# caltech-netlab/adacharge

Hardware: AMD Instinct MI355X
Metric: MPC QP solves/sec whole-node, 54 EVSE x horizon 12; max rate residual vs cvxpy (higher is better)
Workload: dtype f64; 1 GPU; caltech54 (Caltech-shaped, 54 EVSE) x horizon 12, quick_charge + equal_share*1e-12, SOC constraints, batches of 256 independent MPC snapshots (BASELINE.json configs[1]); one step = one acnqp_solve_batches call over 64 such batches per GPU (16384 problems), pinned host buffers in, host buffers out: H2D + kernels + D2H inside the timed region; batch=256, n_evse=54, horizon=12, constraint_type=SOC, parallelism=dp1 (own snapshots per GPU)

## Files before the change

adacharge_amd/backend.py:

```python
from __future__ import annotations

import ctypes as C
import dataclasses
import os
from dataclasses import dataclass
from typing import Optional

import numpy as np

from .builder import CONE_SOC, ProblemBatch, SiteData

_LIB_NAME = "libacn_qp_hip.so"
_LIB_DIR = os.path.join(os.path.dirname(os.path.abspath(__file__)), "lib")

STATUS_UNSET = 0
STATUS_SOLVED = 1
STATUS_MAX_ITER = 2
STATUS_PRIMAL_INFEASIBLE = 3
STATUS_EMPTY_SET = 4
STATUS_SOLVED_INACCURATE = 5
ACCEPTED_STATUSES = (STATUS_SOLVED, STATUS_SOLVED_INACCURATE)
STATUS_NAMES = {
    STATUS_UNSET: "unset",
    STATUS_SOLVED: "optimal",
# ... 122 lines not shown
        ("acnqp_ordered_launch_count", i64, [h]),
        ("acnqp_polish_stats", rc, [h, P(i64), i32]),
        ("acnqp_accel_columns", i32, [h, i32, i32, i32, i32]),
        ("acnqp_route", i32, [h, i32, i32, i32, P(i32)]),
    ]
    for stem, args in (
        ("acnqp_duals", [h, P(_Problems), P(Options), ptr, ptr, ptr, P(_Duals)]),
        ("acnqp_pilots", [h, P(_PilotPlan), ptr, P(_Pilots)]),
        ("acnqp_advance", advance + [P(_Next), ptr]),
        ("acnqp_advance_priced", advance + [P(ClockCost), P(_Next), ptr]),
        ("acnqp_prepare", [h, P(_Problems), P(_PreparePlan), ptr, ptr, P(_PrepareView), ptr]),
    ):
        rows += [(stem + "_host", rc, args), (stem + "_device", rc, args + [stream])]
    introspection = [
        ("acnqp_debug_polish_alongside", i64, [h]),
        ("acnqp_debug_wave_rank", rc, [h, P(i32)]),
        ("acnqp_debug_wave_evse_extent", rc, [h, P(i32)]),
        ("acnqp_debug_order_keys", rc, [h, P(_Problems), P(i32)]),
        ("acnqp_debug_copy_workspace", i64, [h, ptr, i64]),
    ]
    return tuple(r + (True,) for r in rows) + tuple(r + (False,) for r in introspection)


_ABI = _abi()
EXPORTED_SYMBOLS = tuple(name for name, _, _, declared in _ABI if declared)

_lib = None


def library_path() -> str:
# ... 380 lines not shown
        want_y = [False] * n if want_y is None else list(want_y)
        warm = [None] * n if warm is None else list(warm)
        if len(want_y) != n or len(warm) != n:
            raise ValueError("want_y and warm need one entry per batch")
        P, R = (_Problems * n)(), (_Results * n)()
        results, keep = [], []
        for g, batch in enumerate(batches):
            self._check_site(batch)
            P[g], R[g], res, k = self._marshal(batch, pinned_results, warm=warm[g], want_y=bool(want_y[g]))
            results.append(res)
            keep.append(k)
        _check(self._lib.acnqp_solve_batches(self._h, n, P, C.byref(o), R), "acnqp_solve_batches")
        del keep
        return [self._finish(b, r) for b, r in zip(batches, results)]

    def prepare_many(self, batches, pinned_results: bool = True, x_dev_ptrs=None):
        n = len(batches)
        P, R = (_Problems * n)(), (_Results * n)()
        results, keep = [], []
        for g, batch in enumerate(batches):
            self._check_site(batch)
            P[g], R[g], res, k = self._marshal(batch, pinned_results, None if x_dev_ptrs is None else x_dev_ptrs[g])
            results.append(res)
            keep.append(k)

        def run(options: Options):
            _check(self._lib.acnqp_solve_batches(self._h, n, P, C.byref(options), R), "acnqp_solve_batches")
            return results

        run.keep = keep
        return run, results

    def solve_device(self, dev: "DeviceBatch", options: Optional[Options] = None, stream: int = 0, warm_x=None, warm_y=None) -> None:
        o = options if options is not None else default_options()
        if (warm_x is None) != (warm_y is None):
            raise ValueError("warm_x and warm_y go together (both or neither)")
        _want(warm_x, "warm_x", _F8, (dev.B, dev.N, dev.Tm))
# ... 198 lines not shown
        return dict(rank=int(buf[0]), eig_ksteps=int(buf[1]), extent=int(buf[2]))

    def wave_evse_extent(self) -> dict:
        buf = (C.c_int32 * 3)()
        if self._lib.acnqp_debug_wave_evse_extent(self._h, buf) != 0:
            raise RuntimeError("acnqp_debug_wave_evse_extent failed")
        return dict(n_evse=int(buf[0]), evse_ksteps=int(buf[1]), extent=int(buf[2]))

    def order_keys(self, dev: "DeviceBatch") -> np.ndarray:
        keys = np.empty(dev.B, np.int32)
        p = _device_problems(dev)
        if self._lib.acnqp_debug_order_keys(self._h, C.byref(p), keys.ctypes.data_as(C.POINTER(C.c_int32))) != 0:
            raise RuntimeError("acnqp_debug_order_keys failed")
        return keys

    def ordered_launches(self) -> int:
        return int(self._lib.acnqp_ordered_launch_count(self._h))

    def last_kernel_ms(self) -> float:
        return float(self._lib.acnqp_last_kernel_ms(self._h))

    def kernel_times(self, capacity: int = 64):
        buf = (C.c_float * int(capacity))()
        n = int(self._lib.acnqp_kernel_times(self._h, buf, int(capacity)))
        return [float(buf[k]) for k in range(n)]

    def route(self, t_max: int, k_sessions: int, batch: int = 1):
        pol = C.c_int32(0)
        fam = int(self._lib.acnqp_route(self._h, int(t_max), int(k_sessions), int(batch), C.byref(pol)))
        if fam == 0:
# ... 47 lines not shown
```

adacharge_amd/csrc/acn_qp_api.hip:

```cpp
#include <hip/hip_runtime.h>

#include <algorithm>
#include <chrono>
#include <cmath>
#include <cstdint>
#include <cstdio>
#include <cstdlib>
#include <cstring>
#include <initializer_list>
#include <string>
#include <vector>

#include "acn_qp.h"
#include "acn_qp_launch.hpp"
#include "acn_qp_duals.hpp"
#include "acn_qp_pilots.hpp"
#include "acn_qp_advance.hpp"
#include "acn_qp_prepare.hpp"
#include "acn_qp_site.hpp"

namespace {

thread_local std::string g_last_error;

// ... 46 lines not shown
    cap = 0;
  }
};

}

struct acnqp_handle {
  int device = 0;
  acnqp::SiteShape shape;
  std::vector<double> G, limits;
  acnqp::SiteDev site;
  static constexpr int kEvRing = 64;
  hipEvent_t ev_start[kEvRing] = {}, ev_stop[kEvRing] = {};
  long long launches = 0, reported = 0;
  long long ordered_launches = 0;
  static constexpr int kSlots = 4;
  struct Slot { hipStream_t st = nullptr; DevBuf in, out, tin; } slot[kSlots];
  HostBuf small_in, small_out;
  hipEvent_t h2d_done[kSlots] = {nullptr, nullptr, nullptr, nullptr};
  struct Work {
    hipStream_t st; DevBuf buf; DevBuf ord; DevBuf pol; long long used; hipEvent_t last; DevBuf dua;
    hipEvent_t fork = nullptr, join = nullptr;
    void release_events() {
      if (last) (void)hipEventDestroy(last);
      if (fork) (void)hipEventDestroy(fork);
      if (join) (void)hipEventDestroy(join);
      last = fork = join = nullptr;
    }
  };
  std::vector<Work> work;
// ... 79 lines not shown
  static long long stream_workspace(int NP, int CT, int K, int MT, int accel) { return acnqp::stream_workspace(NP, CT, K, MT, accel); }
  static long long long_workspace(int NP, int t_max, int K, int MT, int accel) { return acnqp::long_workspace(NP, acnqp::long_tiles(t_max), K, MT, accel); }
};

int polish_block_doubles(const acnqp_handle* h, const acnqp::Route& rt) {
  static const bool no_polish = std::getenv("ACNQP_NO_POLISH") != nullptr;
  if (no_polish || !rt.polish_shape) return -1;
  const acnqp::SiteShape& s = h->shape;
  const int nrow_site = s.M + s.has_peak;
  const bool two_per_cu = rt.tiled && rt.t_max <= 16 && s.MR == 16 && rt.k_sessions == 1;
  const int blk = acnqp::polish_blocks_that_fit(s.N, rt.t_max, s.Mg, nrow_site, acnqp::polish_max_sess(s.N, rt.k_sessions),
                                                two_per_cu ? 76 * 1024 : 160 * 1024);
  return blk < 2 * nrow_site * (2 * nrow_site + 1) / 2 ? -1 : blk;
}

int solve_batch_device(acnqp_handle* h, const acnqp_problems* p, const acnqp_options* o, acnqp_results* r, hipStream_t st, bool nothing_follows);

}

#include "acn_qp_pipeline.hpp"
#include "acn_qp_post.hpp"
extern "C" {

int32_t acnqp_abi_version(void) { return ACNQP_ABI_VERSION; }

int32_t acnqp_route(acnqp_handle* h, int32_t t_max, int32_t k_sessions, int32_t batch, int32_t* polish) {
  if (polish) *polish = 0;
  if (!h || t_max < 1 || t_max > 4096 || k_sessions < 1 || k_sessions > 4096 || batch < 1) return 0;
  const acnqp::Route r = route_of(h, t_max, k_sessions, batch);
  acnqp_options o;
  acnqp_default_options(&o);
// ... 166 lines not shown
  a.x = r->x; a.status = r->status; a.iters = r->iters; a.pri = r->pri_res; a.dua = r->dua_res; a.obj = r->obj;
  a.eps_abs = o->eps_abs; a.eps_rel = o->eps_rel; a.rho0 = o->rho; a.sigma = o->sigma; a.alpha = o->alpha;
  a.adapt_tol = o->adapt_tol; a.reg_rel = o->reg_rel;
  a.max_iter = o->max_iter; a.check_every = o->check_every; a.adapt_every = o->adapt_every;
  a.peak_scale = d->peak_scale; a.flat_scale = d->flat_scale; a.max_scale = d->max_scale;
  a.accel_mem = std::max(0, o->accel_mem);
  a.stall_iters = o->stall_iters; a.retry_passes = o->retry_passes; a.retry_max_iter = o->retry_max_iter;
  a.retry_rho = o->retry_rho; a.inacc_floor = o->inaccurate_floor;
  a.pbuf_single = 0;
  a.order = nullptr;
  a.queue = nullptr;
  bool own = false;
  for (auto& sl : h->slot) own = own || sl.st == st;
  a.grid_oversub = own ? 4 : 1;
  a.polish_iters = 0; a.polish_stall = 0; a.resume = 0; a.y_for_polish_only = 0; a.pol_rows = 0; a.pol_list = nullptr; a.pol_count = nullptr; a.pol_retired = nullptr; a.count_dev = nullptr;
  return a;
}

hipError_t launch_order_keys(acnqp_handle* h, const acnqp::Route& rt, const acnqp_problems* p, hipStream_t st, int32_t* keys) {
  static const bool by_sessions = [] { const char* e = std::getenv("ACNQP_ORDER_KEY"); return e && std::strcmp(e, "sessions") == 0; }();
  const acnqp::SiteShape& s = h->shape;
  const int g_rows = s.cone == ACNQP_CONE_SOC ? 2 * s.M : s.M;
  const int waves = by_sessions || rt.family == ACNQP_ROUTE_WAVE4 ? 0 : order_key_waves((size_t)s.N, (size_t)p->t_max, (size_t)g_rows);
  if (waves == 0) {
    hipLaunchKernelGGL(session_keys_kernel, dim3((p->batch + 3) / 4), dim3(256), 0, st, p->s_len, p->k_sessions * s.N, p->batch, keys);
    return hipGetLastError();
  }
  OrderKeyArgs ka;
  ka.B = p->batch; ka.N = s.N; ka.Tm = p->t_max; ka.K = p->k_sessions; ka.M = s.M; ka.soc = s.cone == ACNQP_CONE_SOC; ka.has_peak = s.has_peak;
  ka.lb = p->lb; ka.ub = p->ub; ka.s_cap = p->s_cap; ka.peak = p->peak; ka.G = h->site.Gabi; ka.limits = h->site.limabi;
// ... 62 lines not shown
    w.Ghat = h->site.GhatW; w.lam = h->site.lamW; w.fragQ = h->site.fragQW; w.extent = wave_extent_of(h);
    w.evse_ksteps = wave_evse_extent_of(h);
    return acnqp::launch_wave(aa, w, st);
  }
  if (rt.tiled) return rt.t_max <= 16 ? acnqp::launch_tiled_ct1(aa, st) : acnqp::launch_tiled_ct2(aa, st);
  if (rt.stream || rt.lng) {
    acnqp::StreamArgs sa;
    sa.t = aa; sa.work = static_cast<double*>(ws.p); sa.ws_per_problem = ws.per_problem;
    return rt.stream ? acnqp::launch_stream(sa, st) : acnqp::launch_long(sa, st, rt.lds);
  }
  const long long nvar = (long long)rt.site.N * rt.t_max;
  const int nt = nvar <= 4096 ? 256 : (nvar <= 12288 ? 512 : 1024);
  acnqp::GeneralArgs ga;
  ga.t = aa; ga.work = ws.p; ga.ws_per_problem = ws.per_problem; ga.pair_stride = 4;
  return acnqp::launch_general(ga, nt, st);
}

int launch_with_polish(acnqp_handle* h, acnqp_handle::Work* wk, const acnqp::Route& rt, const acnqp::TiledArgs& a, const Workspace& ws,
                       int pol_blk, const acnqp_problems* p, const acnqp_options* o, const acnqp_results* r, hipStream_t st, bool nothing_follows,
                       hipError_t* e) {
  static const bool no_alongside = std::getenv("ACNQP_NO_POLISH_ALONGSIDE") != nullptr;
  static const long long along_polls = [] {
    const char* v = std::getenv("ACNQP_POLISH_ALONGSIDE_SPINS");
    const long long n = v ? std::atoll(v) : (1ll << 21);
    return n < 0 ? 0ll : n;
  }();
  static const int along_grid = [] {
    const char* v = std::getenv("ACNQP_POLISH_ALONGSIDE_GRID");
    const int n = v ? std::atoi(v) : 0;
    return n > 0 && n <= 256 ? n : 16;
// ... 40 lines not shown
    pa.alongside = 0; pa.expected = p->batch; pa.retired = ctr + 3; pa.max_polls = along_polls; pa.taken = h->pol_stats + 16;
    if (alongside) {
      acnqp::PolishArgs pc = pa;
      pc.alongside = 1;
      HIP_TRY(hipStreamWaitEvent(h->aux, wk->fork, 0));
      *e = acnqp::launch_polish(pc, along_grid, h->aux);
      HIP_TRY(hipEventRecord(wk->join, h->aux));
      HIP_TRY(hipStreamWaitEvent(st, wk->join, 0));
    }
    if (*e == hipSuccess) *e = acnqp::launch_polish(pa, pol_grid, st);
  }
  if (*e == hipSuccess) {
    acnqp::TiledArgs a3 = a;
    a3.resume = 1; a3.order = list; a3.count_dev = ctr + 2; a3.queue = ctr + 1;
    a3.warm_x = r->x; a3.warm_y = ybuf;
    a3.ws_by_slot = 1; a3.grid_cap = std::min(p->batch, a.grid_oversub > 1 ? 64 : 2 * h->cus);
    if (!a.ws_by_slot) a3.grid_cap = std::min(a3.grid_cap, a.grid_cap);
    *e = launch_solver(h, rt, a3, ws, st);
  }
  return ACNQP_OK;
}

int solve_batch_device(acnqp_handle* h, const acnqp_problems* p, const acnqp_options* o, acnqp_results* r, hipStream_t st, bool nothing_follows) {
  int rc = check_problem_shapes(h, p, o, r);
  if (rc != ACNQP_OK) return rc;
  if (p->batch == 0) return ACNQP_OK;
  HIP_TRY(hipSetDevice(h->device));
  acnqp::TiledArgs a = tiled_args(h, p, o, r, st);
  (void)hipGetLastError();
  HIP_TRY(hipMemsetAsync(r->status, 0, (size_t)p->batch * sizeof(int32_t), st));
  const int evk = (int)(h->launches % acnqp_handle::kEvRing);
  HIP_TRY(hipEventRecord(h->ev_start[evk], st));
  const acnqp::Route rt = route_of(h, p->t_max, p->k_sessions, p->batch);
  acnqp_handle::Work* wk = h->work_for(st);
  if ((rc = schedule_launch(h, wk, rt, p, st, &a)) != ACNQP_OK) return rc;
  Workspace ws;
  if ((rc = reserve_workspace(wk, rt, st, &a, &ws)) != ACNQP_OK) return rc;
  const int pol_blk = (o->polish_iters > 0 && o->polish_iters < o->max_iter && !a.warm_x) ? polish_block_doubles(h, rt) : -1;
  hipError_t e = hipSuccess;
  if (pol_blk >= 0) {
    if ((rc = launch_with_polish(h, wk, rt, a, ws, pol_blk, p, o, r, st, nothing_follows, &e)) != ACNQP_OK) return rc;
  } else {
    e = launch_solver(h, rt, a, ws, st);
  }
  if (e != hipSuccess) return fail(ACNQP_ERR_HIP, std::string("kernel launch: ") + hipGetErrorString(e));
  HIP_TRY(hipEventRecord(h->ev_stop[evk], st));
  if (wk->last) HIP_TRY(hipEventRecord(wk->last, st));
  ++h->launches;
// ... 29 lines not shown
  HIP_TRY(hipSetDevice(h->device));
  HIP_TRY(hipDeviceSynchronize());
  int32_t v[16] = {0};
  HIP_TRY(hipMemcpy(v, h->pol_stats, sizeof(v), hipMemcpyDeviceToHost));
  for (int k = 0; k < capacity && k < 16; ++k) out[k] = v[k];
  return ACNQP_OK;
}

extern "C" int64_t acnqp_debug_polish_alongside(acnqp_handle* h) {
  if (!h || hipSetDevice(h->device) != hipSuccess || hipDeviceSynchronize() != hipSuccess) return -1;
  int32_t v = 0;
  if (hipMemcpy(&v, h->pol_stats + 16, sizeof v, hipMemcpyDeviceToHost) != hipSuccess) return -1;
  if (hipMemset(h->pol_stats + 16, 0, sizeof v) != hipSuccess) return -1;
  return v;
}

extern "C" int acnqp_debug_wave_rank(acnqp_handle* h, int32_t* out) {
  if (!h || !out) return -1;
  const int ext = wave_extent_of(h);
  out[0] = h->site.rank; out[1] = h->site.eig_ksteps; out[2] = ext > 0 ? ext : h->shape.MR / 4;
  return 0;
}

extern "C" int acnqp_debug_order_keys(acnqp_handle* h, const acnqp_problems* p, int32_t* keys_out) {
  if (!h || !p || !keys_out || p->batch < 0 || p->t_max < 1 || p->k_sessions < 1) return -1;
  if (p->batch == 0) return 0;
  if (!p->lb || !p->ub || !p->s_off || !p->s_len || !p->s_cap || !p->horizon) return -1;
  if (hipSetDevice(h->device) != hipSuccess) return -1;
  int32_t* keys = nullptr;
  if (hipMalloc((void**)&keys, (size_t)p->batch * sizeof(int32_t)) != hipSuccess) return -1;
// ... 128 lines not shown
```

adacharge_amd/csrc/acn_qp_common.hpp:

```cpp
#pragma once
#include <hip/hip_runtime.h>
#include <stdint.h>

#include "acn_qp_check.hpp"

namespace acnqp {

#ifdef ACNQP_STAMPS
__device__ unsigned long long g_stamps[1024 * 16 * 12];
#define STAMP(slot)                                                                    \
  do {                                                                                 \
    unsigned long long _t;                                                             \
    __builtin_amdgcn_sched_barrier(0);                                                 \
    asm volatile("s_memtime %0\n\ts_waitcnt lgkmcnt(0)" : "=s"(_t)::"memory");         \
    __builtin_amdgcn_sched_barrier(0);                                                 \
    st_acc[slot] += _t - st_prev;                                                      \
    st_prev = _t;                                                                      \
  } while (0)
#else
#define STAMP(slot) do {} while (0)
#endif

#ifndef ACNQP_GUARD_MAX
#define ACNQP_GUARD_MAX 120
// ... 26 lines not shown
  double *pri, *dua, *obj;
  double eps_abs, eps_rel, rho0, sigma, alpha, adapt_tol, reg_rel;
  double peak_scale, flat_scale, max_scale;
  int max_iter, check_every, adapt_every;
  int accel_mem;
  int stall_iters, retry_passes, retry_max_iter;
  double inacc_floor, retry_rho;
  int pbuf_single;
  int polish_iters, resume;
  int polish_stall;
  int y_for_polish_only;
  int pol_rows;
  int32_t *pol_list, *pol_count;
  int32_t* pol_retired;
  const int32_t* count_dev;
  int ws_by_slot;
  int grid_oversub;
  int grid_cap;
};

typedef const __attribute__((address_space(4))) TiledArgs* KernargPtr;

__device__ inline int queue_length(const TiledArgs& a) {
  if (a.count_dev == nullptr) return a.B;
  const int n = *a.count_dev;
  return n < a.B ? n : a.B;
}
__device__ inline int queue_next(int32_t* queue, int B, int round, int* slot_lds) {
  if (queue == nullptr) return round == 0 && (int)blockIdx.x < B ? (int)blockIdx.x : -1;
  if (threadIdx.x == 0) *slot_lds = atomicAdd(queue, 1);
// ... 160 lines not shown
```

adacharge_amd/csrc/acn_qp_pipeline.hpp:

```cpp
#pragma once
#include <algorithm>
#include <cstddef>
#include <cstdlib>
#include <vector>

namespace acnqp {

inline size_t al256(size_t b) { return (b + 255) & ~(size_t)255; }

struct ChunkLayout {
  size_t lb, ub, q, pd, hz, so, sl, sc, eq, pk, lf, dc, df, wx, wy, in_total;
  size_t x, st, it, pr, du, ob, y, out_total;
  ChunkLayout(size_t cn, size_t N, size_t Tm, size_t K, size_t Mg, bool peak, bool flat, bool mx, bool warm, bool want_y) {
    size_t o = 0;
    lb = o; o += al256(cn * N * Tm * 8);
    ub = o; o += al256(cn * N * Tm * 8);
    q = o;  o += al256(cn * N * Tm * 8);
    pd = o; o += al256(cn * 8);
    hz = o; o += al256(cn * 4);
    so = o; o += al256(cn * K * N * 4);
    sl = o; o += al256(cn * K * N * 4);
    sc = o; o += al256(cn * K * N * 8);
    eq = o; o += al256(cn);
    pk = o; o += al256(peak ? cn * Tm * 8 : 0);
    lf = o; o += al256(flat ? cn * 8 : 0);
    dc = o; o += al256(mx ? cn * 8 : 0);
    df = o; o += al256(mx ? cn * 8 : 0);
    wx = o; o += al256(warm ? cn * N * Tm * 8 : 0);
    wy = o; o += al256(warm ? cn * Mg * Tm * 8 : 0);
    in_total = o;
    o = 0;
    x = o;  o += al256(cn * N * Tm * 8);
    st = o; o += al256(cn * 4);
    it = o; o += al256(cn * 4);
    pr = o; o += al256(cn * 8);
    du = o; o += al256(cn * 8);
    ob = o; o += al256(cn * 8);
    y = o;  o += al256(want_y ? cn * Mg * Tm * 8 : 0);
    out_total = o;
  }
};

struct PlanEnv {
  long long chunk = 0;
  const char* plan = nullptr;
  bool ramp = true;
};

inline long long chunk_cap_by_memory(size_t N, size_t Tm, size_t K) {
  const size_t per_problem = 4 * N * Tm * 8 + K * N * 16 + Tm * 8 + 96;
  return (long long)((size_t)1024 * 1024 * 1024 / std::max<size_t>(per_problem, 1));
}

inline std::vector<long long> plan_chunk_caps(long long total, long long want, long long by_mem, bool wave, bool uniform,
                                              const PlanEnv& env) {
  if (env.chunk > 0) want = env.chunk;
  long long cap = std::max<long long>(1, std::min(want, by_mem));
  if (cap >= 512) cap -= cap % 512;
  std::vector<long long> caps;
  if (env.ramp && wave && uniform) {
    if (env.plan) {
      for (const char* q = env.plan; *q;) { caps.push_back(std::max<long long>(1, std::atoll(q))); while (*q && *q != ',') ++q; if (*q == ',') ++q; }
    } else if (total >= 2048 && cap >= 2048) {
      const long long k = (total + cap - 1) / cap - 1;
      long long c = total / (k + 1);
      c = std::max<long long>(2048, std::min(cap, c - c % 512));
      caps.push_back(c / 4);
      caps.push_back(c / 2);
      for (long long i = 0; i < k; ++i) caps.push_back(c);
    }
    caps.push_back(std::max<long long>(1, total));
  } else if (env.ramp && cap >= 1024) {
    caps = {cap / 4, cap / 2, cap};
  } else {
    caps = {cap};
  }
  return caps;
// ... 176 lines not shown
    qt = o; o += al256((size_t)T->n_horizons * nv * 8);
    total = o;
  }
};

struct BatchShape { long long batch; int t_max, k_sessions; bool warm, want_y; };
struct Piece { int g; long long lo, n, pos; };
struct Scatter { int g; size_t lo, n, pos; const char* host; size_t st, it, pr, du, ob; };

struct Call {
  const acnqp_problems* P = nullptr;
  const acnqp_table* T = nullptr;
  acnqp_results* R = nullptr;
  std::vector<BatchShape> bs;
  std::vector<Scatter> scatter;
};

void device_views(const ChunkLayout& L, char* di, char* dq, const acnqp::SiteShape& s, size_t cn, const BatchShape& b,
                  acnqp_problems* dp, acnqp_results* dr) {
  dp->batch = (int32_t)cn; dp->t_max = b.t_max; dp->k_sessions = b.k_sessions;
  dp->lb = reinterpret_cast<const double*>(di + L.lb);
  dp->ub = reinterpret_cast<const double*>(di + L.ub);
  dp->q = reinterpret_cast<const double*>(di + L.q);
  dp->pdiag = reinterpret_cast<const double*>(di + L.pd);
  dp->horizon = reinterpret_cast<const int32_t*>(di + L.hz);
  dp->s_off = reinterpret_cast<const int32_t*>(di + L.so);
  dp->s_len = reinterpret_cast<const int32_t*>(di + L.sl);
  dp->s_cap = reinterpret_cast<const double*>(di + L.sc);
  dp->s_eq = reinterpret_cast<const uint8_t*>(di + L.eq);
  dp->peak = s.has_peak ? reinterpret_cast<const double*>(di + L.pk) : nullptr;
  dp->lf = s.has_flat ? reinterpret_cast<const double*>(di + L.lf) : nullptr;
// ... 18 lines not shown
    total += b.batch;
    uniform = uniform && b.t_max == bs[0].t_max && b.k_sessions == bs[0].k_sessions && b.warm == bs[0].warm && b.want_y == bs[0].want_y;
  }
  std::vector<std::vector<Piece>> chunks;
  std::vector<long long> caps;
  long long fill = 0, cap = 0;
  const BatchShape* cur = nullptr;
  for (int g = 0; g < (int)bs.size(); ++g) {
    const BatchShape& b = bs[g];
    for (long long lo = 0; lo < b.batch;) {
      if (!cur || b.t_max != cur->t_max || b.k_sessions != cur->k_sessions || b.warm != cur->warm || b.want_y != cur->want_y || fill >= cap) {
        chunks.emplace_back();
        cur = &b; fill = 0;
        if (caps.empty() || !uniform) {
          const acnqp::Route rt = acnqp::route_for(h->shape, b.t_max, b.k_sessions, (int)std::min<long long>(total, acnqp::kRouteAnyBatch), route_switches());
          caps = acnqp::plan_chunk_caps(total, rt.chunk_want(), acnqp::chunk_cap_by_memory((size_t)h->shape.N, (size_t)b.t_max, (size_t)b.k_sessions),
                                        rt.wv > 0, uniform, env);
        }
        cap = acnqp::chunk_cap(caps, chunks.size() - 1);
      }
      const long long n = std::min(b.batch - lo, cap - fill);
      chunks.back().push_back({g, lo, n, fill});
      fill += n; lo += n;
    }
  }
  return chunks;
}

int fill_dense(acnqp_handle* h, const Call& call, size_t c, const std::vector<Piece>& pcs, const ChunkLayout& L,
               acnqp_handle::Slot& S, char* hs) {
  const acnqp::SiteShape& s = h->shape;
  const BatchShape& b = call.bs[pcs[0].g];
// ... 13 lines not shown
    else H2D(field, base, elem, per);                                                                           \
  } while (0)
    H2D(lb, L.lb, 8, nv);
    H2D(ub, L.ub, 8, nv);
    H2D(q, L.q, 8, nv);
    H2S(pdiag, L.pd, 8, 1);
    H2S(horizon, L.hz, 4, 1);
    H2S(s_off, L.so, 4, ns);
    H2S(s_len, L.sl, 4, ns);
    H2S(s_cap, L.sc, 8, ns);
    H2S(s_eq, L.eq, 1, 1);
    if (s.has_peak) H2S(peak, L.pk, 8, Tm);
    if (s.has_flat) H2S(lf, L.lf, 8, 1);
    if (s.has_max) { H2S(dc, L.dc, 8, 1); H2S(dfloor, L.df, 8, 1); }
    if (b.warm) { H2D(warm_x, L.wx, 8, nv); H2D(warm_y, L.wy, 8, Mg * Tm); }
#undef H2S
#undef H2D
  }
  if (hs) HIP_TRY(hipMemcpyAsync(di + L.pd, hs + L.pd, L.wx - L.pd, hipMemcpyHostToDevice, S.st));
  if (chain) HIP_TRY(hipEventRecord(h->h2d_done[c % acnqp_handle::kSlots], S.st));
  return ACNQP_OK;
}

int fill_table(acnqp_handle* h, const Call& call, const Piece& pc, const ChunkLayout& L, const TableLayout& TL, acnqp_handle::Slot& S) {
  const acnqp::SiteShape& s = h->shape;
  const acnqp_table* T = call.T;
  const size_t N = s.N, Tm = T->t_max, K = T->k_sessions, nv = N * Tm;
  const long long lo = pc.lo, cn = pc.n, s0 = TL.s0, ns = TL.ns, r0 = TL.r0, nr = TL.nr;
  char* di = static_cast<char*>(S.in.p);
  char* dt = static_cast<char*>(S.tin.p);
// ... 27 lines not shown
  ea.lb = reinterpret_cast<double*>(di + L.lb); ea.ub = reinterpret_cast<double*>(di + L.ub); ea.q = reinterpret_cast<double*>(di + L.q);
  ea.so = reinterpret_cast<int32_t*>(di + L.so); ea.sl = reinterpret_cast<int32_t*>(di + L.sl); ea.sc = reinterpret_cast<double*>(di + L.sc);
  hipLaunchKernelGGL(table_expand_kernel, dim3((unsigned)cn), dim3(256), 0, S.st, ea);
  return ACNQP_OK;
}

int run_call(acnqp_handle* h, Call& call, const acnqp_options* o) {
  const acnqp::SiteShape& s = h->shape;
  const size_t N = s.N, Mg = s.Mg;
  const bool table = call.T != nullptr;
  acnqp::PlanEnv env;
  if (const char* e = std::getenv("ACNQP_CHUNK")) env.chunk = std::atoll(e);
  env.plan = std::getenv("ACNQP_PLAN");
  static const bool ramp = std::getenv("ACNQP_NO_RAMP") == nullptr;
  env.ramp = ramp;
  const std::vector<std::vector<Piece>> chunks = split_call(h, call.bs, env);
  auto layout = [&](const std::vector<Piece>& pcs) {
    const BatchShape& b = call.bs[pcs[0].g];
    return ChunkLayout((size_t)(pcs.back().pos + pcs.back().n), N, b.t_max, b.k_sessions, Mg, s.has_peak, s.has_flat, s.has_max, b.warm, b.want_y);
  };
  constexpr size_t kSmallCap = (size_t)256 << 20;
  std::vector<size_t> in_off(chunks.size()), out_off(chunks.size());
  size_t in_sum = 0, out_sum = 0;
  for (size_t c = 0; c < chunks.size() && !table; ++c) {
    const ChunkLayout L = layout(chunks[c]);
    in_off[c] = in_sum; in_sum += L.wx - L.pd;
    out_off[c] = out_sum; out_sum += L.y - L.st;
  }
  static const bool no_stage = std::getenv("ACNQP_NO_STAGING") != nullptr;
  const bool staged = !table && !no_stage && in_sum + out_sum <= kSmallCap;
  if (staged) {
    HIP_TRY(h->small_in.reserve(in_sum));
    HIP_TRY(h->small_out.reserve(out_sum));
  }
  for (size_t c = 0; c < chunks.size(); ++c) {
    acnqp_handle::Slot& S = h->slot[c % acnqp_handle::kSlots];
    const std::vector<Piece>& pcs = chunks[c];
    const BatchShape& b = call.bs[pcs[0].g];
    const size_t cn = (size_t)(pcs.back().pos + pcs.back().n), Tm = b.t_max;
    const ChunkLayout L = layout(pcs);
    const TableLayout TL = table ? TableLayout(call.T, pcs[0].lo, pcs[0].n, N * Tm) : TableLayout();
    if (L.in_total > S.in.cap || L.out_total > S.out.cap || TL.total > S.tin.cap) HIP_TRY(hipStreamSynchronize(S.st));
    HIP_TRY(S.in.reserve(L.in_total));
    HIP_TRY(S.out.reserve(L.out_total));
    if (table) HIP_TRY(S.tin.reserve(TL.total));
    char* di = static_cast<char*>(S.in.p);
    char* dq = static_cast<char*>(S.out.p);
    char* hs = staged ? static_cast<char*>(h->small_in.p) + in_off[c] - L.pd : nullptr;
    char* ho = staged ? static_cast<char*>(h->small_out.p) + out_off[c] - L.st : nullptr;
    int rc = table ? fill_table(h, call, pcs[0], L, TL, S) : fill_dense(h, call, c, pcs, L, S, hs);
    if (rc != ACNQP_OK) return rc;
    acnqp_problems dp;
    acnqp_results dr;
    device_views(L, di, dq, s, cn, b, &dp, &dr);
    rc = solve_batch_device(h, &dp, o, &dr, S.st, c + 1 == chunks.size());
    if (rc != ACNQP_OK) return rc;
    if (staged) HIP_TRY(hipMemcpyAsync(ho + L.st, dq + L.st, L.y - L.st, hipMemcpyDeviceToHost, S.st));
    for (const Piece& pc : pcs) {
      const acnqp_results& r = call.R[pc.g];
      const size_t lo = (size_t)pc.lo, n = (size_t)pc.n, pos = (size_t)pc.pos;
#define D2H(field, base, elem, per)                                                                          \
  HIP_TRY(hipMemcpyAsync(reinterpret_cast<char*>(r.field) + lo * (per) * (elem), dq + (base) + pos * (per) * (elem), \
                         n * (per) * (elem), hipMemcpyDeviceToHost, S.st))
      D2H(x, L.x, 8, N * Tm);
      if (staged) {
        call.scatter.push_back(Scatter{pc.g, lo, n, pos, ho, L.st, L.it, L.pr, L.du, L.ob});
      } else {
        D2H(status, L.st, 4, 1);
        D2H(iters, L.it, 4, 1);
        D2H(pri_res, L.pr, 8, 1);
        D2H(dua_res, L.du, 8, 1);
        D2H(obj, L.ob, 8, 1);
      }
      if (b.want_y) D2H(y, L.y, 8, Mg * Tm);
#undef D2H
      if (r.x_dev)
        HIP_TRY(hipMemcpyAsync(r.x_dev + lo * N * Tm, dq + L.x + pos * N * Tm * 8, n * N * Tm * 8, hipMemcpyDeviceToDevice, S.st));
    }
  }
// ... 38 lines not shown
```

adacharge_amd/csrc/acn_qp_route.hpp:

```cpp
#pragma once
#include <algorithm>

#include "acn_qp.h"

namespace acnqp {

constexpr int kRouteMaxK = 4;
constexpr int kRouteWaveTS = 12;

inline int padded_rows(int cone, int M, int has_peak, int has_flat, int has_max) {
  return (cone == ACNQP_CONE_SOC ? 8 * ((M + 3) / 4) : M) + (has_peak ? 1 : 0) + (has_flat ? 1 : 0) + (has_max ? 1 : 0);
}

struct SiteShape {
  int N = 0, M = 0, Mg = 0, MR = 0;
  int cone = 0, has_peak = 0, has_flat = 0, has_max = 0;
  int NP() const { return N <= 64 ? 64 : 16 * ((N + 15) / 16); }
};

inline SiteShape site_shape(int N, int M, int cone, int has_peak, int has_flat, int has_max) {
  SiteShape s;
  s.N = N; s.M = M; s.cone = cone;
  s.has_peak = has_peak ? 1 : 0; s.has_flat = has_flat ? 1 : 0; s.has_max = has_max ? 1 : 0;
  s.Mg = (cone == ACNQP_CONE_SOC ? 2 * M : M) + s.has_peak + s.has_flat + s.has_max;
// ... 31 lines not shown
inline bool stream_shape(const SiteShape& s, int t_max) { return s.N > 64 && t_max <= 48; }
inline bool long_shape(const SiteShape& s, int t_max, int k_sessions, const RouteSwitches& sw) {
  return !sw.no_long && !tiled_shape(s, t_max, k_sessions) && !stream_shape(s, t_max) && t_max <= 288 && s.MR <= 32;
}

struct Route {
  int family = 0;
  int wv = 0;
  bool tiled = false, stream = false, lng = false, lds = false, on_chip = false;
  bool polish_shape = false;
  SiteShape site;
  int t_max = 0, k_sessions = 0;

  long long chunk_want() const { return wv > 0 ? 8192 : (tiled ? 1024 : 2048); }

  template <class Kn> int accel_cap() const {
    if (wv > 0) return Kn::wave_accel();
    if (tiled) return Kn::tiled_accel(site.MR / 16, (t_max + 15) / 16, site.NP(), k_sessions);
    if (stream) return Kn::stream_accel();
    if (lng) return Kn::long_accel();
    return Kn::general_accel();
  }

  template <class Kn> long long workspace_doubles(int accel_req) const {
    if (tiled) return 0;
    const int accel = std::min(std::max(0, accel_req), accel_cap<Kn>());
    if (stream) return Kn::stream_workspace(site.NP(), (t_max + 15) / 16, k_sessions, site.MR / 16, accel);
    if (lng) return Kn::long_workspace(site.NP(), t_max, k_sessions, site.MR / 16, accel);
    const long long n = (long long)site.N * t_max, mt = (long long)site.MR * t_max, Dn = n + mt;
    return 7 * n + 8 * mt + 3LL * k_sessions * site.N + 8 + 2 * Dn + ((1 + 2LL * accel) * Dn * 4 + 7) / 8 + 2;
// ... 26 lines not shown
```

adacharge_amd/csrc/acn_qp_wave.hpp:

```cpp
#pragma once
#include <type_traits>

#include "acn_qp_common.hpp"

namespace acnqp {

constexpr int kWaveTS = 12;
constexpr int kWaveXS = 17;
constexpr int kWaveNW = 4;
constexpr int kWaveAM = 5;

struct WaveLds {
  int fragp, fragx, fragq, rowc, wave0, wstride;
  int xt, rowd, aah, snap, hist, total;
  int xch;
  int xs;
  __host__ __device__ WaveLds(int accel_mem, int npw = 1, int mt = 1, int tsv = kWaveTS) {
    int o = 0;
    fragp = o; o += mt * 16 * 64;
    fragx = o; o += 4 * 4 * mt * 64;
    fragq = o; o += mt * mt * 2 * 4 * 64;
    rowc = o;  o += mt * (16 + 16 + 8);
    wave0 = o;
    int w = 0;
// ... 16 lines not shown
    const int pos = (int)blockIdx.x * kWaveNW + wave;
    return round == 0 && pos < B ? pos : -1;
  }
  int v = 0;
  if (lane == 0) v = atomicAdd(queue, 1);
  const int pos = __builtin_amdgcn_readfirstlane(v);
  return pos < B ? pos : -1;
}

__device__ inline void wave_lds_sync() {
  __builtin_amdgcn_fence(__ATOMIC_RELEASE, "wavefront");
  __builtin_amdgcn_wave_barrier();
  __builtin_amdgcn_fence(__ATOMIC_ACQUIRE, "wavefront");
}

template <int AM, int NPW, int TSV, int MT, bool PROX, int EK = 0, int NE = 0>
__global__ __launch_bounds__(kWaveNW * 64, 1) void admm_wave_kernel(const TiledArgs A_kernarg) {
  static_assert(NPW == 1 || NPW == 2 || NPW == 4, "one, two or four waves per problem");
  static_assert((TSV == 12 && MT == 1) || (TSV == 6 && MT == 2 && NPW >= 2), "instantiated: 12 periods x one row tile, 6 periods x two row tiles");
  using M = Mfma<double>;
  using vec4 = typename M::vec4;
  typedef double real;
  constexpr int TS = TSV, XS = TSV > 8 ? kWaveXS : 9, XC = TSV > 8 ? 16 : 8;
  constexpr int SR = 4 * MT, KS = 4 * MT;
  constexpr int EKS = EK > 0 ? EK : KS, ET = (EKS + 3) / 4;
  static_assert(EKS <= KS, "eigen extent");
  constexpr int NKS = NE > 0 ? NE : 16;
  static_assert(NKS <= 16, "EVSE extent");
#define EKOF(m) (EKS - 4 * (m) < 4 ? EKS - 4 * (m) : 4)
#define BIGC (scalar_const(1e300))
// ... 291 lines not shown
#pragma unroll
    for (int t = 0; t < TS; ++t) {
      f1 = fmax(f1, fabs(qv[t]));
      f2 = fmax(f2, ubv[t]);
      if (!((swm >> t) & 1u)) f3 = fmax(f3, fmax(fabs(lbv[t]), fabs(ubv[t])));
    }
    f1 = wave_max<real>(f1); f2 = wave_max<real>(f2); f3 = wave_max<real>(f3);
    { real f[3] = {f1, f2, f3}; pu_max(f, 3); f1 = f[0]; f2 = f[1]; f3 = f[2]; }
    plain_windows = uniform_scalar(f3) == 0.0;
    qnorm = uniform_scalar(f1);
    pd = uniform_scalar(effective_pdiag<real>(pd_user, A.reg_rel, qnorm, uniform_scalar(f2), A.horizon[b], PROX && ((lfb > 0.0) | (dcb > 0.0))));
    if (__any(empty_set)) {
#pragma unroll
      for (int t = 0; t < TS; ++t)
        if (act && tb + t < Tm) A.x[((size_t)b * N + lane) * Tm + tb + t] = 0;
      if (A.y_out && !A.y_for_polish_only && half == 0)
        for (int k = lane; k < A.Mg * Tm; k += 64) A.y_out[(size_t)b * A.Mg * Tm + k] = 0;
      if (lane == 0 && half == 0) {
        A.status[b] = 4; A.iters[b] = 0;
        A.pri[b] = 1e300; A.dua[b] = 1e300; A.obj[b] = 0;
      }
      break;
    }
  }

  real z2[SR], y2[SR], gx[SR];
#pragma unroll
  for (int r = 0; r < SR; ++r) { z2[r] = 0; y2[r] = 0; gx[r] = 0; }

  rho = uniform_scalar(rho);
// ... 655 lines not shown
    STAMP(7);
  }
  it_total += it;
  if (lane == 0 && half == 0) A.iters[b] = it_total;
  if (pass == 0 || status_rank(status) > status_rank(best_status)) {
    best_status = status;
    real ol = 0;
    int lane_o = lane;
    asm volatile("" : "+v"(lane_o));
#pragma unroll
    for (int t = 0; t < TS; ++t)
      if (lane_o < N && tb + t < Tm) {
        A.x[((size_t)b * N + lane_o) * Tm + tb + t] = z1[t];
        ol += (0.5 * pd_user * z1[t] + qv[t]) * z1[t];
      }
    if (A.y_out && (!A.y_for_polish_only || status == kStatusPolish)) {
      const real* RS = static_cast<const real*>(A.rowscale);
      const int g_o = lane_o >> 4, t_o = lane_o & 15;
#pragma unroll
      for (int r = 0; r < SR; ++r) {
        const int j = 16 * (r >> 2) + M::rowof(g_o, r & 3);
        const int ja = A.rowabi[j];
        if (ja >= 0 && t_o < TS && tb + t_o < Tm) A.y_out[((size_t)b * A.Mg + ja) * Tm + tb + t_o] = y2[r] * RS[j];
      }
    }
    if (status == kStatusPolish) __threadfence();
    ol = wave_sum<real>(ol);
    { real o1[1] = {ol}; pu_sum(o1, 1); ol = o1[0]; }
    if (lane == 0 && half == 0) {
      A.status[b] = xbroken ? 0 : status;
// ... 31 lines not shown
```

Measured before the change: 1.040 million QP solves/s.

## Write solution x directly to pinned host memory from the wave kernel

When the caller's x output buffer is pinned host memory, the single-wave solver kernel now stores each problem's solution straight into the host-mapped pointer, and so does a small follow-up kernel for polished problems. This skips the per-chunk x device-to-host memcpy. The chunk planner also gets a direct-mode split (small ramp-up chunks, then equal large ones) to overlap with this. The risk is that zero-copy PCIe writes from the kernel are slow or uncoalesced and lengthen kernel time. It adds a pointer table to each chunk's input.

```diff
diff --git a/adacharge_amd/backend.py b/adacharge_amd/backend.py
--- a/adacharge_amd/backend.py
+++ b/adacharge_amd/backend.py
@@ -160,6 +160,7 @@
         rows += [(stem + "_host", rc, args), (stem + "_device", rc, args + [stream])]
     introspection = [
         ("acnqp_debug_polish_alongside", i64, [h]),
+        ("acnqp_debug_direct_x", i64, [h]),
         ("acnqp_debug_wave_rank", rc, [h, P(i32)]),
         ("acnqp_debug_wave_evse_extent", rc, [h, P(i32)]),
         ("acnqp_debug_order_keys", rc, [h, P(_Problems), P(i32)]),
@@ -570,13 +571,17 @@
         del keep
         return [self._finish(b, r) for b, r in zip(batches, results)]
 
-    def prepare_many(self, batches, pinned_results: bool = True, x_dev_ptrs=None):
+    def prepare_many(self, batches, pinned_results=True, x_dev_ptrs=None, warm=None):
         n = len(batches)
+        warm = [None] * n if warm is None else list(warm)
+        pinned = [bool(pinned_results)] * n if isinstance(pinned_results, (bool, np.bool_)) else [bool(v) for v in pinned_results]
+        if len(pinned) != n or len(warm) != n:
+            raise ValueError("pinned_results and warm need one entry per batch")
         P, R = (_Problems * n)(), (_Results * n)()
         results, keep = [], []
         for g, batch in enumerate(batches):
             self._check_site(batch)
-            P[g], R[g], res, k = self._marshal(batch, pinned_results, None if x_dev_ptrs is None else x_dev_ptrs[g])
+            P[g], R[g], res, k = self._marshal(batch, pinned[g], None if x_dev_ptrs is None else x_dev_ptrs[g], warm=warm[g])
             results.append(res)
             keep.append(k)
 
@@ -805,6 +810,9 @@
             raise RuntimeError("acnqp_debug_order_keys failed")
         return keys
 
+    def direct_x(self) -> int:
+        return int(self._lib.acnqp_debug_direct_x(self._h))
+
     def ordered_launches(self) -> int:
         return int(self._lib.acnqp_ordered_launch_count(self._h))
 
diff --git a/adacharge_amd/csrc/acn_qp_api.hip b/adacharge_amd/csrc/acn_qp_api.hip
--- a/adacharge_amd/csrc/acn_qp_api.hip
+++ b/adacharge_amd/csrc/acn_qp_api.hip
@@ -84,6 +84,7 @@
   hipEvent_t ev_start[kEvRing] = {}, ev_stop[kEvRing] = {};
   long long launches = 0, reported = 0;
   long long ordered_launches = 0;
+  long long direct_x_last = 0;
   static constexpr int kSlots = 4;
   struct Slot { hipStream_t st = nullptr; DevBuf in, out, tin; } slot[kSlots];
   HostBuf small_in, small_out;
@@ -193,7 +194,8 @@
   return blk < 2 * nrow_site * (2 * nrow_site + 1) / 2 ? -1 : blk;
 }
 
-int solve_batch_device(acnqp_handle* h, const acnqp_problems* p, const acnqp_options* o, acnqp_results* r, hipStream_t st, bool nothing_follows);
+int solve_batch_device(acnqp_handle* h, const acnqp_problems* p, const acnqp_options* o, acnqp_results* r, hipStream_t st, bool nothing_follows,
+                       double* const* x_host = nullptr);
 
 }
 
@@ -390,6 +392,7 @@
   for (auto& sl : h->slot) own = own || sl.st == st;
   a.grid_oversub = own ? 4 : 1;
   a.polish_iters = 0; a.polish_stall = 0; a.resume = 0; a.y_for_polish_only = 0; a.pol_rows = 0; a.pol_list = nullptr; a.pol_count = nullptr; a.pol_retired = nullptr; a.count_dev = nullptr;
+  a.x_host = nullptr;
   return a;
 }
 
@@ -482,6 +485,18 @@
   acnqp::GeneralArgs ga;
   ga.t = aa; ga.work = ws.p; ga.ws_per_problem = ws.per_problem; ga.pair_stride = 4;
   return acnqp::launch_general(ga, nt, st);
+}
+
+__global__ __launch_bounds__(256) void pol_x_to_host_kernel(const int32_t* list, const int32_t* count, int B, int nv, const double* x,
+                                                            double* const* x_host) {
+  const int n = min(*count, B);
+  for (int pos = blockIdx.x; pos < n; pos += gridDim.x) {
+    const int b = list[pos];
+    if (b < 0 || b >= B) continue;
+    double* const dst = x_host[b];
+    if (dst == nullptr) continue;
+    for (int k = threadIdx.x; k < nv; k += blockDim.x) dst[k] = x[(size_t)b * nv + k];
+  }
 }
 
 int launch_with_polish(acnqp_handle* h, acnqp_handle::Work* wk, const acnqp::Route& rt, const acnqp::TiledArgs& a, const Workspace& ws,
@@ -552,14 +567,21 @@
     acnqp::TiledArgs a3 = a;
     a3.resume = 1; a3.order = list; a3.count_dev = ctr + 2; a3.queue = ctr + 1;
     a3.warm_x = r->x; a3.warm_y = ybuf;
+    a3.x_host = nullptr;
     a3.ws_by_slot = 1; a3.grid_cap = std::min(p->batch, a.grid_oversub > 1 ? 64 : 2 * h->cus);
     if (!a.ws_by_slot) a3.grid_cap = std::min(a3.grid_cap, a.grid_cap);
     *e = launch_solver(h, rt, a3, ws, st);
   }
+  if (*e == hipSuccess && a.x_host != nullptr) {
+    hipLaunchKernelGGL(pol_x_to_host_kernel, dim3((unsigned)std::min(p->batch, 64)), dim3(256), 0, st, list, ctr + 2, p->batch,
+                       s.N * p->t_max, r->x, a.x_host);
+    *e = hipGetLastError();
+  }
   return ACNQP_OK;
 }
 
-int solve_batch_device(acnqp_handle* h, const acnqp_problems* p, const acnqp_options* o, acnqp_results* r, hipStream_t st, bool nothing_follows) {
+int solve_batch_device(acnqp_handle* h, const acnqp_problems* p, const acnqp_options* o, acnqp_results* r, hipStream_t st, bool nothing_follows,
+                       double* const* x_host) {
   int rc = check_problem_shapes(h, p, o, r);
   if (rc != ACNQP_OK) return rc;
   if (p->batch == 0) return ACNQP_OK;
@@ -570,6 +592,8 @@
   const int evk = (int)(h->launches % acnqp_handle::kEvRing);
   HIP_TRY(hipEventRecord(h->ev_start[evk], st));
   const acnqp::Route rt = route_of(h, p->t_max, p->k_sessions, p->batch);
+  if (x_host != nullptr && !rt.direct_x()) return fail(ACNQP_ERR_INVALID, "direct x on a route that cannot store it");
+  a.x_host = x_host;
   acnqp_handle::Work* wk = h->work_for(st);
   if ((rc = schedule_launch(h, wk, rt, p, st, &a)) != ACNQP_OK) return rc;
   Workspace ws;
@@ -629,6 +653,8 @@
   if (hipMemset(h->pol_stats + 16, 0, sizeof v) != hipSuccess) return -1;
   return v;
 }
+
+extern "C" int64_t acnqp_debug_direct_x(acnqp_handle* h) { return h ? (int64_t)h->direct_x_last : -1; }
 
 extern "C" int acnqp_debug_wave_rank(acnqp_handle* h, int32_t* out) {
   if (!h || !out) return -1;
diff --git a/adacharge_amd/csrc/acn_qp_common.hpp b/adacharge_amd/csrc/acn_qp_common.hpp
--- a/adacharge_amd/csrc/acn_qp_common.hpp
+++ b/adacharge_amd/csrc/acn_qp_common.hpp
@@ -64,6 +64,7 @@
   int32_t *pol_list, *pol_count;
   int32_t* pol_retired;
   const int32_t* count_dev;
+  double* const* x_host;
   int ws_by_slot;
   int grid_oversub;
   int grid_cap;
diff --git a/adacharge_amd/csrc/acn_qp_pipeline.hpp b/adacharge_amd/csrc/acn_qp_pipeline.hpp
--- a/adacharge_amd/csrc/acn_qp_pipeline.hpp
+++ b/adacharge_amd/csrc/acn_qp_pipeline.hpp
@@ -9,9 +9,9 @@
 inline size_t al256(size_t b) { return (b + 255) & ~(size_t)255; }
 
 struct ChunkLayout {
-  size_t lb, ub, q, pd, hz, so, sl, sc, eq, pk, lf, dc, df, wx, wy, in_total;
+  size_t lb, ub, q, pd, hz, so, sl, sc, eq, pk, lf, dc, df, xh, wx, wy, in_total;
   size_t x, st, it, pr, du, ob, y, out_total;
-  ChunkLayout(size_t cn, size_t N, size_t Tm, size_t K, size_t Mg, bool peak, bool flat, bool mx, bool warm, bool want_y) {
+  ChunkLayout(size_t cn, size_t N, size_t Tm, size_t K, size_t Mg, bool peak, bool flat, bool mx, bool warm, bool want_y, bool direct = false) {
     size_t o = 0;
     lb = o; o += al256(cn * N * Tm * 8);
     ub = o; o += al256(cn * N * Tm * 8);
@@ -26,6 +26,7 @@
     lf = o; o += al256(flat ? cn * 8 : 0);
     dc = o; o += al256(mx ? cn * 8 : 0);
     df = o; o += al256(mx ? cn * 8 : 0);
+    xh = o; o += al256(direct ? cn * sizeof(double*) : 0);
     wx = o; o += al256(warm ? cn * N * Tm * 8 : 0);
     wy = o; o += al256(warm ? cn * Mg * Tm * 8 : 0);
     in_total = o;
@@ -45,6 +46,7 @@
   long long chunk = 0;
   const char* plan = nullptr;
   bool ramp = true;
+  bool direct = false;
 };
 
 inline long long chunk_cap_by_memory(size_t N, size_t Tm, size_t K) {
@@ -61,6 +63,17 @@
   if (env.ramp && wave && uniform) {
     if (env.plan) {
       for (const char* q = env.plan; *q;) { caps.push_back(std::max<long long>(1, std::atoll(q))); while (*q && *q != ',') ++q; if (*q == ',') ++q; }
+    } else if (env.direct && total >= 2048 && cap >= 2048) {
+      long long m = 1, u = 0;
+      for (;; ++m) {
+        u = (total + 4 + 3 * m) / (5 + 3 * m);
+        if (3 * u <= cap) break;
+      }
+      const long long f = total - 3 * u * m;
+      caps.push_back(std::max<long long>(1, f / 5));
+      caps.push_back(std::max<long long>(1, 2 * f / 5));
+      caps.push_back(std::max<long long>(1, f - f / 5 - 2 * f / 5));
+      for (long long i = 0; i < m; ++i) caps.push_back(3 * u);
     } else if (total >= 2048 && cap >= 2048) {
       const long long k = (total + cap - 1) / cap - 1;
       long long c = total / (k + 1);
@@ -267,7 +280,19 @@
   acnqp_results* R = nullptr;
   std::vector<BatchShape> bs;
   std::vector<Scatter> scatter;
+  std::vector<double*> xdst;
 };
+
+double* direct_destination(const double* x) {
+  static const bool off = std::getenv("ACNQP_NO_DIRECT_X") != nullptr;
+  if (off || x == nullptr) return nullptr;
+  hipPointerAttribute_t at;
+  if (hipPointerGetAttributes(&at, x) != hipSuccess) {
+    (void)hipGetLastError();
+    return nullptr;
+  }
+  return at.type == hipMemoryTypeHost ? static_cast<double*>(at.devicePointer) : nullptr;
+}
 
 void device_views(const ChunkLayout& L, char* di, char* dq, const acnqp::SiteShape& s, size_t cn, const BatchShape& b,
                   acnqp_problems* dp, acnqp_results* dr) {
@@ -316,8 +341,10 @@
         cur = &b; fill = 0;
         if (caps.empty() || !uniform) {
           const acnqp::Route rt = acnqp::route_for(h->shape, b.t_max, b.k_sessions, (int)std::min<long long>(total, acnqp::kRouteAnyBatch), route_switches());
+          acnqp::PlanEnv e = env;
+          e.direct = env.direct && rt.direct_x();
           caps = acnqp::plan_chunk_caps(total, rt.chunk_want(), acnqp::chunk_cap_by_memory((size_t)h->shape.N, (size_t)b.t_max, (size_t)b.k_sessions),
-                                        rt.wv > 0, uniform, env);
+                                        rt.wv > 0, uniform, e);
         }
         cap = acnqp::chunk_cap(caps, chunks.size() - 1);
       }
@@ -361,6 +388,11 @@
     if (s.has_flat) H2S(lf, L.lf, 8, 1);
     if (s.has_max) { H2S(dc, L.dc, 8, 1); H2S(dfloor, L.df, 8, 1); }
     if (b.warm) { H2D(warm_x, L.wx, 8, nv); H2D(warm_y, L.wy, 8, Mg * Tm); }
+    if (hs && L.xh != L.wx) {
+      double** tab = reinterpret_cast<double**>(hs + L.xh) + pos;
+      double* const dst = call.xdst[pc.g];
+      for (size_t i = 0; i < n; ++i) tab[i] = dst ? dst + (lo + i) * nv : nullptr;
+    }
 #undef H2S
 #undef H2D
   }
@@ -418,16 +450,32 @@
   env.plan = std::getenv("ACNQP_PLAN");
   static const bool ramp = std::getenv("ACNQP_NO_RAMP") == nullptr;
   env.ramp = ramp;
+  h->direct_x_last = 0;
+  call.xdst.assign(call.bs.size(), nullptr);
+  env.direct = !table && !call.bs.empty();
+  for (size_t g = 0; g < call.bs.size() && !table; ++g) {
+    call.xdst[g] = call.bs[g].batch > 0 ? direct_destination(call.R[g].x) : nullptr;
+    env.direct = env.direct && (call.xdst[g] != nullptr || call.bs[g].batch == 0);
+  }
   const std::vector<std::vector<Piece>> chunks = split_call(h, call.bs, env);
-  auto layout = [&](const std::vector<Piece>& pcs) {
+  std::vector<char> direct(chunks.size(), 0);
+  for (size_t c = 0; c < chunks.size() && !table; ++c) {
+    const std::vector<Piece>& pcs = chunks[c];
     const BatchShape& b = call.bs[pcs[0].g];
-    return ChunkLayout((size_t)(pcs.back().pos + pcs.back().n), N, b.t_max, b.k_sessions, Mg, s.has_peak, s.has_flat, s.has_max, b.warm, b.want_y);
+    if (!route_of(h, b.t_max, b.k_sessions, (int)(pcs.back().pos + pcs.back().n)).direct_x()) continue;
+    for (const Piece& pc : pcs) direct[c] = direct[c] || call.xdst[pc.g] != nullptr;
+  }
+  auto layout = [&](size_t c) {
+    const std::vector<Piece>& pcs = chunks[c];
+    const BatchShape& b = call.bs[pcs[0].g];
+    return ChunkLayout((size_t)(pcs.back().pos + pcs.back().n), N, b.t_max, b.k_sessions, Mg, s.has_peak, s.has_flat, s.has_max, b.warm, b.want_y,
+                       direct[c] != 0);
   };
   constexpr size_t kSmallCap = (size_t)256 << 20;
   std::vector<size_t> in_off(chunks.size()), out_off(chunks.size());
   size_t in_sum = 0, out_sum = 0;
   for (size_t c = 0; c < chunks.size() && !table; ++c) {
-    const ChunkLayout L = layout(chunks[c]);
+    const ChunkLayout L = layout(c);
     in_off[c] = in_sum; in_sum += L.wx - L.pd;
     out_off[c] = out_sum; out_sum += L.y - L.st;
   }
@@ -436,13 +484,15 @@
   if (staged) {
     HIP_TRY(h->small_in.reserve(in_sum));
     HIP_TRY(h->small_out.reserve(out_sum));
+  } else {
+    std::fill(direct.begin(), direct.end(), 0);
   }
   for (size_t c = 0; c < chunks.size(); ++c) {
     acnqp_handle::Slot& S = h->slot[c % acnqp_handle::kSlots];
     const std::vector<Piece>& pcs = chunks[c];
     const BatchShape& b = call.bs[pcs[0].g];
     const size_t cn = (size_t)(pcs.back().pos + pcs.back().n), Tm = b.t_max;
-    const ChunkLayout L = layout(pcs);
+    const ChunkLayout L = layout(c);
     const TableLayout TL = table ? TableLayout(call.T, pcs[0].lo, pcs[0].n, N * Tm) : TableLayout();
     if (L.in_total > S.in.cap || L.out_total > S.out.cap || TL.total > S.tin.cap) HIP_TRY(hipStreamSynchronize(S.st));
     HIP_TRY(S.in.reserve(L.in_total));
@@ -457,7 +507,8 @@
     acnqp_problems dp;
     acnqp_results dr;
     device_views(L, di, dq, s, cn, b, &dp, &dr);
-    rc = solve_batch_device(h, &dp, o, &dr, S.st, c + 1 == chunks.size());
+    double* const* x_host = direct[c] ? reinterpret_cast<double* const*>(di + L.xh) : nullptr;
+    rc = solve_batch_device(h, &dp, o, &dr, S.st, c + 1 == chunks.size(), x_host);
     if (rc != ACNQP_OK) return rc;
     if (staged) HIP_TRY(hipMemcpyAsync(ho + L.st, dq + L.st, L.y - L.st, hipMemcpyDeviceToHost, S.st));
     for (const Piece& pc : pcs) {
@@ -466,7 +517,8 @@
 #define D2H(field, base, elem, per)                                                                          \
   HIP_TRY(hipMemcpyAsync(reinterpret_cast<char*>(r.field) + lo * (per) * (elem), dq + (base) + pos * (per) * (elem), \
                          n * (per) * (elem), hipMemcpyDeviceToHost, S.st))
-      D2H(x, L.x, 8, N * Tm);
+      if (direct[c] && call.xdst[pc.g]) h->direct_x_last += (long long)n;
+      else D2H(x, L.x, 8, N * Tm);
       if (staged) {
         call.scatter.push_back(Scatter{pc.g, lo, n, pos, ho, L.st, L.it, L.pr, L.du, L.ob});
       } else {
diff --git a/adacharge_amd/csrc/acn_qp_route.hpp b/adacharge_amd/csrc/acn_qp_route.hpp
--- a/adacharge_amd/csrc/acn_qp_route.hpp
+++ b/adacharge_amd/csrc/acn_qp_route.hpp
@@ -69,6 +69,8 @@
 
   long long chunk_want() const { return wv > 0 ? 8192 : (tiled ? 1024 : 2048); }
 
+  bool direct_x() const { return wv == 1; }
+
   template <class Kn> int accel_cap() const {
     if (wv > 0) return Kn::wave_accel();
     if (tiled) return Kn::tiled_accel(site.MR / 16, (t_max + 15) / 16, site.NP(), k_sessions);
diff --git a/adacharge_amd/csrc/acn_qp_wave.hpp b/adacharge_amd/csrc/acn_qp_wave.hpp
--- a/adacharge_amd/csrc/acn_qp_wave.hpp
+++ b/adacharge_amd/csrc/acn_qp_wave.hpp
@@ -54,6 +54,17 @@
   __builtin_amdgcn_fence(__ATOMIC_ACQUIRE, "wavefront");
 }
 
+__device__ __attribute__((always_inline)) inline void wave_x_to_host(const double* xt, int xs, int n, int Tm, double* dst) {
+  const int lane = threadIdx.x & 63;
+  int row = lane / Tm, col = lane - row * Tm;
+  const int drow = 64 / Tm, dcol = 64 - drow * Tm;
+  for (int k = lane; k < n; k += 64) {
+    dst[k] = xt != nullptr ? xt[row * xs + col] : 0.0;
+    row += drow; col += dcol;
+    if (col >= Tm) { col -= Tm; ++row; }
+  }
+}
+
 template <int AM, int NPW, int TSV, int MT, bool PROX, int EK = 0, int NE = 0>
 __global__ __launch_bounds__(kWaveNW * 64, 1) void admm_wave_kernel(const TiledArgs A_kernarg) {
   static_assert(NPW == 1 || NPW == 2 || NPW == 4, "one, two or four waves per problem");
@@ -375,6 +386,10 @@
 #pragma unroll
       for (int t = 0; t < TS; ++t)
         if (act && tb + t < Tm) A.x[((size_t)b * N + lane) * Tm + tb + t] = 0;
+      if constexpr (NPW == 1) {
+        double* const xh = A.x_host != nullptr ? A.x_host[b] : nullptr;
+        if (xh != nullptr) wave_x_to_host(nullptr, 0, N * Tm, Tm, xh);
+      }
       if (A.y_out && !A.y_for_polish_only && half == 0)
         for (int k = lane; k < A.Mg * Tm; k += 64) A.y_out[(size_t)b * A.Mg * Tm + k] = 0;
       if (lane == 0 && half == 0) {
@@ -1060,6 +1075,16 @@
         A.x[((size_t)b * N + lane_o) * Tm + tb + t] = z1[t];
         ol += (0.5 * pd_user * z1[t] + qv[t]) * z1[t];
       }
+    if constexpr (NPW == 1) {
+      double* const xh = A.x_host != nullptr ? A.x_host[b] : nullptr;
+      if (xh != nullptr && status != kStatusPolish) {
+        __builtin_amdgcn_wave_barrier();
+#pragma unroll
+        for (int t = 0; t < TS; ++t) XT[lane_o * XS + t] = z1[t];
+        wave_lds_sync();
+        wave_x_to_host(XT, XS, N * Tm, Tm, xh);
+      }
+    }
     if (A.y_out && (!A.y_for_polish_only || status == kStatusPolish)) {
       const real* RS = static_cast<const real*>(A.rowscale);
       const int g_o = lane_o >> 4, t_o = lane_o & 15;
```

Result: faster. 1.068 million QP solves/s, median of 6 (+2.7%).
